# tspooner/rl_markets

Measured on NVIDIA H100. Metric: env steps/sec (batched LOBs), higher is better.
Workload: dtype f64

## Files before the change

rl_markets_b200/csrc/rlm_env.cuh:

```cuda
#pragma once
#include <cuda_runtime.h>
#include <math.h>
#include "rlm_types.h"

__constant__ DevParams P;

#define LLMIN ((long long)0x8000000000000000ull)
#ifdef RLM_ROLL_LEVELS
#define LEVEL_UNROLL _Pragma("unroll 1")
#else
#define LEVEL_UNROLL _Pragma("unroll")
#endif

__device__ __forceinline__ double pkey(double p) { return rint(p * 10000.0); }

__device__ __forceinline__ long long d2ll_x86(double d) {
  if (!(d >= -9223372036854775808.0 && d < 9223372036854775808.0)) return LLMIN;
  return (long long)d;
}

static_assert((RLM_MAX_BANDS & (RLM_MAX_BANDS - 1)) == 0, "the band search halves RLM_MAX_BANDS");
__device__ __noinline__ int to_ticks(double price, int* err, int* band_hint = nullptr) {
  const VenueD& V = P.venue;
  if (price < V.px[0]) { *err |= ERR_TICK_RANGE; return 0; }
  int k = 0;
  const int hk = band_hint ? *band_hint : -1;
  if ((unsigned)hk < (unsigned)(RLM_MAX_BANDS - 1) && !(price < V.px[hk]) && price < V.px[hk + 1]) {
    k = hk;
  } else {
#pragma unroll
    for (int step = RLM_MAX_BANDS / 2; step >= 1; step >>= 1)
      if (!(price < V.px[k + step])) k += step;
    if (band_hint) *band_hint = k;
  }
  int ticks = V.cum_full[k];
  double tsp = V.ts[k];
  int it = k;
#pragma unroll 1
  while (it < V.n && price + V.ts[it] / 2.0 > V.px[it]) {
    double ub;
    if (it == V.n - 1 || price < V.px[it + 1]) ub = price + tsp / 2.0;
    else ub = V.px[it + 1];
    const double inv = V.inv_ts[it];
    const double q = (inv != 0.0) ? (ub - V.px[it]) * inv : (ub - V.px[it]) / V.ts[it];
    ticks = (int)((double)ticks + q);
    ++it;
  }
  return ticks;
}

__device__ __noinline__ double to_price(int ticks, int* err) {
  const VenueD& V = P.venue;
  if (ticks < V.tts_tick[0]) { *err |= ERR_TICK_RANGE; return 0.0; }
  if (!(ticks > V.tts_tick[0])) return 0.0;
  int k = 0;
#pragma unroll
  for (int step = RLM_MAX_BANDS / 2; step >= 1; step >>= 1)
    if (ticks >= V.tts_tick[k + step]) k += step;
  double price = V.cum_price[k];
  if (ticks > V.tts_tick[k]) price += ((double)ticks - (double)V.tts_tick[k]) * V.ts[k];
  return price;
}

__device__ __forceinline__ bool market_is_open(const EnvHdr& e) {
  return ((long long)e.time_ms > P.venue.open_lo) && ((long long)e.time_ms < P.venue.close_hi);
}
__device__ __forceinline__ bool is_terminal(const EnvHdr& e) {
  return (!market_is_open(e)) || ((e.last_date != 0) && (e.date != e.last_date));
}

__device__ __forceinline__ long long ord_remaining(const OrderD& o) {
  long long r = o.size - o.executed;
  return r > 0 ? r : 0;
}
__device__ __forceinline__ bool ord_is_executed(const OrderD& o) { return o.executed >= o.size; }

__device__ __noinline__ long long ord_do_transaction(OrderD& o, long long volume) {
  o.transactions += (int)volume;
  long long remaining_volume = volume - o.q_head;
  if (remaining_volume > 0) {
    o.q_head = 0;
    if (ord_remaining(o) <= remaining_volume) {
      o.executed = o.size;
      remaining_volume -= o.size;
    } else {
      o.executed += remaining_volume;
      remaining_volume = 0;
    }
  } else {
    o.q_head -= volume;
  }
  return remaining_volume > 0 ? remaining_volume : 0;
}

__device__ __noinline__ void ord_do_cancellation(OrderD& o, long long volume) {
  if (o.q_tail == 0) {
    o.q_head -= volume;
  } else {
    double total = (double)(o.q_head + o.q_tail);
    o.q_head = d2ll_x86((double)o.q_head - ceil((double)(volume * o.q_head) / total));
    o.q_tail = d2ll_x86((double)o.q_tail - floor((double)(volume * o.q_tail) / total));
  }
  if (o.q_head < 0) {
    o.q_tail = (long long)((unsigned long long)o.q_tail + (unsigned long long)o.q_head);
    o.q_head = 0;
  }
  if (o.q_tail < 0) o.q_tail = 0;
}

__device__ long long side_volume(const SideD& s, double price) {
  if (!s.has_cur) return 0;
  double k = pkey(price);
  long long v = 0;
  LEVEL_UNROLL
  for (int l = 0; l < RLM_DEPTH; ++l)
    if (pkey(s.px[l]) == k) v = s.vol[l];
  return v;
}
__device__ long long side_last_volume(const SideD& s, double price) {
  if (!s.has_last) return 0;
  double k = pkey(price);
  long long v = 0;
  LEVEL_UNROLL
  for (int l = 0; l < RLM_DEPTH; ++l)
    if (pkey(s.last_px[l]) == k) v = s.last_vol[l];
  return v;
}

__device__ __noinline__ void side_reset(SideD& s) {
  s.n_transacted = 0; s.obs_value = 0.0; s.obs_volume = 0;
  s.total_vol = 0; s.last_total_vol = 0;
  for (int l = 0; l < RLM_DEPTH; ++l) { s.px[l] = 0.0; s.last_px[l] = 0.0; s.vol[l] = 0; s.last_vol[l] = 0; }
  s.has_cur = 0; s.has_last = 0;
  s.ord.live = 0;
}

__device__ __noinline__ void side_replace_order(SideD& s, double price, long long size, int* err) {
  if (price <= 0 || size <= 0) { *err |= ERR_BAD_PRICE; s.ord.live = 0; return; }
  OrderD& o = s.ord;
  o.live = 1; o.price = price; o.size = size;
  o.q_head = side_volume(s, price);
  o.q_tail = 0; o.executed = 0; o.transactions = 0; o.initial_queue = o.q_head;
}

__device__ __noinline__ void side_update_order(SideD& s, long long transaction_volume) {
  OrderD& o = s.ord;
  if (!o.live) return;
  if (ord_is_executed(o)) { o.live = 0; return; }
  long long lv = side_last_volume(s, o.price);
  if (lv == 0) return;
  long long v = side_volume(s, o.price);
  if (v == 0) { o.q_head = 0; o.q_tail = 0; return; }
  long long vol_diff = lv - v;
  if (vol_diff >= 0) {
    long long cancelled = vol_diff - transaction_volume;
    if (cancelled > 0) ord_do_cancellation(o, cancelled);
  } else {
    o.q_tail += vol_diff;
  }
}
// ... 135 lines not shown
}
__device__ __forceinline__ double win_back(const EnvHdr& e, const double* ring, int w) {
  int i = (e.w_count[w] == P.win_size[w]) ? e.w_head[w] : 0;
  return ring[P.win_off[w] + i];
}
__device__ __forceinline__ double win_std(const EnvHdr& e, int w) {
  double v = e.w_s[w] / (double)((unsigned long long)((long long)e.w_count[w] - 1));
  return v > 0 ? sqrt(v) : 0.0;
}

__device__ __noinline__ double get_reward(const EnvHdr& e) {
  double r = 0.0;
  long long ap = e.position < 0 ? -e.position : e.position;
  int abs_pos = (int)ap;
  switch (P.reward_measure) {
    case RLM_REWARD_NONE: break;
    case RLM_REWARD_PNL: r = e.pnl_step; break;
    case RLM_REWARD_PNL_DAMPED: r = e.pnl_step - (double)P.damping * fmax(0.0, e.momentum_pnl_step); break;
    case RLM_REWARD_SPREAD: r = e.pnl_step / e.w_mean[W_SPREAD]; break;
    case RLM_REWARD_NORMED:
      if (!(e.w_count[W_PNLUP] == P.win_size[W_PNLUP] && e.w_count[W_PNLDN] == P.win_size[W_PNLDN])) r = 0.0;
      else {
        double u = e.w_mean[W_PNLUP], d = e.w_mean[W_PNLDN];
        double su = win_std(e, W_PNLUP), sd = win_std(e, W_PNLDN);
        double numer = (u * sd - d * su), denom = (su + sd);
        if (isnan(numer) || isinf(numer)) numer = 0.0;
        if (isnan(denom) || isinf(denom)) denom = 0.0;
        r = (fabs(denom) < 1e-5) ? numer : (numer / denom);
      }
      break;
    case RLM_REWARD_LOVOL: r = (double)e.lo_vol_step; break;
    case RLM_REWARD_MM_LINEAR: r = (double)(-P.pos_weight * (float)abs_pos); r += (double)P.pnl_weight * e.pnl_step; break;
    case RLM_REWARD_MM_EXP:
      r = -pow(1.0 - exp((double)(P.pos_weight * (float)abs_pos)), 2.0); r += (double)P.pnl_weight * e.pnl_step; break;
    case RLM_REWARD_MM_DIV:
      if (e.pnl_step > 0) r = e.pnl_step / fmax(1.0, (double)abs_pos);
      else r = e.pnl_step;
      break;
  }
  return r * 100.0;
}

__device__ __noinline__ void clear_inventory(EnvHdr& e) {
  long long size = -e.position;
  Fill f; f.volume = 0; f.proxy = 0.0; f.value = 0.0;
  double mip = m_midprice(e);
  if (size > 0) f = side_walk<true>(e.side[0], mip, size);
  else if (size < 0) f = side_walk<false>(e.side[1], mip, size);
  e.position += f.volume;
  e.pnl_step += f.proxy;
  e.lo_vol_step += (int)(f.volume < 0 ? -f.volume : f.volume);
  e.ep_pnl += f.value;
  if (f.volume > 0) e.market_buys++;
  else if (f.volume < 0) e.market_sells++;
}

__device__ __noinline__ void place_orders(EnvHdr& e, int al, int bl) {
  e.ask_level = al; e.bid_level = bl;
  if (P.l2p_book) {
    e.ask_quote = to_price(to_ticks(e.side[0].px[0], &e.err, &e.tk_band) + al, &e.err);
    e.bid_quote = to_price(to_ticks(e.side[1].px[0], &e.err, &e.tk_band) - bl, &e.err);
  } else {
    double tp = e.tp_val, half_spd = fmax(0.0, e.w_mean[W_SPREAD] / 2.0);
    e.ask_quote = to_price(to_ticks(tp + (double)al * half_spd, &e.err, &e.tk_band), &e.err);
    e.bid_quote = to_price(to_ticks(tp - (double)bl * half_spd, &e.err, &e.tk_band), &e.err);
  }
  side_replace_order(e.side[0], e.ask_quote, P.order_size, &e.err);
  side_replace_order(e.side[1], e.bid_quote, P.order_size, &e.err);
}

__device__ __noinline__ void do_action(EnvHdr& e, int action) {
  int al, bl;
  switch (action) {
    case 0: al = 1; bl = 1; break;
    case 1: clear_inventory(e); al = e.ask_level; bl = e.bid_level; break;
    case 2: al = 2; bl = 2; break;
    case 3: al = 3; bl = 3; break;
    case 4: al = 0; bl = 2; break;
    case 5: al = 2; bl = 0; break;
    case 6: al = 1; bl = 4; break;
    case 7: al = 4; bl = 1; break;
    case 8: al = 5; bl = 5; break;
    default: return;
  }
  place_orders(e, al, bl);
}

__device__ __noinline__ void update_stats(EnvHdr& e) {
  e.ts_total++;
  bool has_ask = e.side[0].ord.live, has_bid = e.side[1].ord.live;
  if (has_ask) e.ts_ask++;
  if (has_bid) e.ts_bid++;
  if (has_ask && has_bid) e.ts_both++;
  if (e.position != 0) e.ts_pos++;
  if (e.position > 0) e.ts_long++;
  else if (e.position < 0) e.ts_short++;
}

__device__ __noinline__ void update_book_profiles(EnvHdr& e, const rlm_tick_msg& m) {
  e.last_date = e.date;
  e.date = m.date;
  e.time_ms = m.time_ms;
  side_apply_changes(e.side[0], m.ask_px, m.ask_vol, m, &e.err);
  side_apply_changes(e.side[1], m.bid_px, m.bid_vol, m, &e.err);
  if (e.side[0].has_last && e.side[1].has_last && !(pkey(e.side[0].last_px[0]) == 0.0) && !(pkey(e.side[1].last_px[0]) == 0.0)) {
    double mp = m_midprice(e);
    bool ok = (m_spread(e) >= 0.0) && (mp > 0.0) && (fabs(mp - m_last_midprice(e)) < mp);
    if (!ok) e.err |= ERR_INVALID_STATE;
  }
}

__device__ __noinline__ void next_state_tail(EnvHdr& e, const Fill& au, const Fill& bu, double* pushv) {
  Fill as = adverse_selection(e);
  e.pnl_step += au.proxy + bu.proxy + as.proxy;
  long long asabs = as.volume < 0 ? -as.volume : as.volume;
  e.lo_vol_step += (int)(bu.volume - au.volume + asabs);
  e.ep_pnl += au.value + bu.value + as.value;
  e.position += bu.volume + au.volume + as.volume;
  check_orders(e);
  double mid = m_midprice(e);
  long long mpt;
  if (mid == e.tk_px && mid > 0.0) mpt = e.tk_ticks;
  else { const int t = to_ticks(mid, &e.err, &e.tk_band); mpt = t; e.tk_px = mid; e.tk_ticks = t; }
  double mpm = mid - m_last_midprice(e), sp = m_spread(e);
  pushv[W_MID] = (double)mpt;
  pushv[W_VLT] = (double)mpt;
  pushv[W_VNUM] = e.side[0].obs_value + e.side[1].obs_value;
  pushv[W_VDEN] = (double)(e.side[0].obs_volume + e.side[1].obs_volume);
  pushv[W_SPREAD] = fmax(0.0, sp);
  pushv[W_TP] = P.tp_is_micro ? m_microprice(e) : mid;
  pushv[W_ASKTX] = (double)e.side[0].obs_volume;
  pushv[W_BIDTX] = (double)e.side[1].obs_volume;
  e.ewma_up = (P.ewma_alpha * fmax(0.0, mpm)) + ((1 - P.ewma_alpha) * e.ewma_up);
  e.ewma_dn = (P.ewma_alpha * fabs(fmin(0.0, mpm))) + ((1 - P.ewma_alpha) * e.ewma_dn);
  e.n_ticks++;
}

__device__ __forceinline__ void check_valid_state(EnvHdr& e) {
  if (e.side[0].has_last && e.side[1].has_last && !(pkey(e.side[0].last_px[0]) == 0.0) && !(pkey(e.side[1].last_px[0]) == 0.0)) {
    double mp = m_midprice(e);
    bool ok = (m_spread(e) >= 0.0) && (mp > 0.0) && (fabs(mp - m_last_midprice(e)) < mp);
    if (!ok) e.err |= ERR_INVALID_STATE;
  }
}

__device__ __noinline__ void next_state_scalar(EnvHdr& e, const rlm_tick_msg& m, double* pushv) {
  double mp = m_midprice(e);
  Fill au = side_apply_transactions<true>(e.side[0], m, mp, true);
  Fill bu = side_apply_transactions<false>(e.side[1], m, mp, true);
  update_book_profiles(e, m);
  next_state_tail(e, au, bu, pushv);
}

__device__ __noinline__ void next_state_warp(EnvHdr& e, const rlm_tick_msg& m, double* pushv, Fill* fills, int lane) {
  int* serr = (int*)(fills + 2);
  if (lane < 2) {
    const double mp = m_midprice(e);
    serr[lane] = 0;
    fills[lane] = (lane == 0) ? side_apply_transactions<true>(e.side[0], m, mp, true)
                              : side_apply_transactions<false>(e.side[1], m, mp, true);
  }
  __syncwarp();
  if (lane < 2) side_apply_changes(e.side[lane], lane == 0 ? m.ask_px : m.bid_px, lane == 0 ? m.ask_vol : m.bid_vol, m, &serr[lane]);
  __syncwarp();
  if (lane == 0) {
    e.last_date = e.date; e.date = m.date; e.time_ms = m.time_ms;
    e.err |= serr[0] | serr[1];
    check_valid_state(e);
    next_state_tail(e, fills[0], fills[1], pushv);
  }
}

__device__ __forceinline__ bool needs_multi(const EnvHdr& e, const rlm_tick_msg& m) { return (m.flags & 3) != 0 || e.tick_open != 0 || e.txn != 0; }
__device__ __forceinline__ void tick_tx_append(EnvHdr& e, const rlm_tick_msg& m) {
  for (int i = 0; i < m.n_tx && i < RLM_N_TX_MAX; ++i) {
    if (e.txn >= RLM_TX_CAP) { e.err |= ERR_BAD_PRICE; break; }
    e.tx_px[e.txn] = m.tx_px[i]; e.tx_vol[e.txn] = m.tx_vol[i]; e.txn++;
  }
}
__device__ __noinline__ bool update_book_profiles_multi(EnvHdr& e, const rlm_tick_msg& m, bool with_tx) {
  if (m.flags & RLM_TICK_TX_MORE) { if (with_tx && !e.tick_open) tick_tx_append(e, m); return false; }
  if (!e.tick_open) {
    if (with_tx) tick_tx_append(e, m); else e.txn = 0;
    side_stash(e.side[0]);
    side_stash(e.side[1]);
  }
  e.last_date = e.date;
  e.date = m.date;
  e.time_ms = m.time_ms;
  side_apply_row(e.side[0], m.ask_px, m.ask_vol, e.tx_px, e.tx_vol, e.txn, &e.err);
  side_apply_row(e.side[1], m.bid_px, m.bid_vol, e.tx_px, e.tx_vol, e.txn, &e.err);
  if (m.flags & RLM_TICK_PARTIAL) { e.tick_open = 1; return false; }
  e.tick_open = 0;
  e.txn = 0;
  return true;
}
__device__ __noinline__ bool next_state_multi(EnvHdr& e, const rlm_tick_msg& m, double* pushv) {
  if (m.flags & RLM_TICK_TX_MORE) { if (!e.tick_open) tick_tx_append(e, m); return false; }
  if (!e.tick_open) {
    tick_tx_append(e, m);
    const double mp = m_midprice(e);
    const Fill au = side_apply_transactions_n<true>(e.side[0], e.tx_px, e.tx_vol, e.txn, mp);
    const Fill bu = side_apply_transactions_n<false>(e.side[1], e.tx_px, e.tx_vol, e.txn, mp);
    e.tick_au.volume = au.volume; e.tick_au.proxy = au.proxy; e.tick_au.value = au.value;
    e.tick_bu.volume = bu.volume; e.tick_bu.proxy = bu.proxy; e.tick_bu.value = bu.value;
    side_stash(e.side[0]);
    side_stash(e.side[1]);
  }
  e.last_date = e.date;
  e.date = m.date;
  e.time_ms = m.time_ms;
  side_apply_row(e.side[0], m.ask_px, m.ask_vol, e.tx_px, e.tx_vol, e.txn, &e.err);
  side_apply_row(e.side[1], m.bid_px, m.bid_vol, e.tx_px, e.tx_vol, e.txn, &e.err);
  if (m.flags & RLM_TICK_PARTIAL) { e.tick_open = 1; return false; }
  e.tick_open = 0;
  e.txn = 0;
  check_valid_state(e);
  Fill au, bu;
  au.volume = e.tick_au.volume; au.proxy = e.tick_au.proxy; au.value = e.tick_au.value;
  bu.volume = e.tick_bu.volume; bu.proxy = e.tick_bu.proxy; bu.value = e.tick_bu.value;
  next_state_tail(e, au, bu, pushv);
  return true;
}

__device__ __forceinline__ double ulb_ref(double val, double lb, double ub) {
  const double m = (ub < val) ? ub : val;
  return (m < lb) ? lb : m;
}

__device__ __forceinline__ bool var_tick_args(const EnvHdr& e, const double* ring, int v, double& x0, double& x1) {
  switch (v) {
    case RLM_VAR_SPD: x0 = e.side[0].px[0]; x1 = e.side[1].px[0]; return true;
    case RLM_VAR_MPM: x0 = win_front(e, ring, W_MID); x1 = win_back(e, ring, W_MID); return true;
    case RLM_VAR_A_DIST: if (!e.side[0].ord.live) return false; x0 = e.side[0].ord.price; x1 = e.side[0].px[0]; return true;
    case RLM_VAR_B_DIST: if (!e.side[1].ord.live) return false; x0 = e.side[1].px[0]; x1 = e.side[1].ord.price; return true;
  }
  return false;
}
__device__ __forceinline__ double var_from_ticks(int v, int t0, int t1) {
  switch (v) {
    case RLM_VAR_SPD: return ulb_ref((double)(t0 - t1), 0.0, 20.0);
    case RLM_VAR_MPM: return ulb_ref((double)(t0 - t1), -10.0, 10.0);
  }
  return (double)t0 - (double)t1;
}

__device__ __noinline__ double get_variable(EnvHdr& e, const double* ring, int v) {
  switch (v) {
    case RLM_VAR_POS: return (double)e.position / (double)P.order_size;
    case RLM_VAR_SPD: {
      double d = (double)(to_ticks(e.side[0].px[0], &e.err, &e.tk_band) - to_ticks(e.side[1].px[0], &e.err, &e.tk_band));
      return ulb_ref(d, 0.0, 20.0);
    }
    case RLM_VAR_MPM: {
      double d = (double)(to_ticks(win_front(e, ring, W_MID), &e.err, &e.tk_band) - to_ticks(win_back(e, ring, W_MID), &e.err, &e.tk_band));
      return ulb_ref(d, -10.0, 10.0);
    }
    case RLM_VAR_IMB: {
      double v_a = (double)e.side[0].total_vol, v_b = (double)e.side[1].total_vol;
      return ((v_a + v_b) > 0 ? 5.0 * (v_b - v_a) / (v_b + v_a) : 0.0);
    }
    case RLM_VAR_SVL: {
      double q_a = e.w_sum[W_ASKTX], q_b = e.w_sum[W_BIDTX];
      return ((q_a + q_b) > 0 ? 5.0 * (q_b - q_a) / (q_a + q_b) : 0.0);
    }
    case RLM_VAR_VOL: return ulb_ref(5.0 * win_std(e, W_VLT), 0.0, 10.0);
    case RLM_VAR_RSI: {
      double u = e.ewma_up, d = e.ewma_dn;
      return (u + d) != 0.0 ? 5.0 * (u - d) / (u + d) : 0.0;
    }
    case RLM_VAR_VWAP: {
      double d = e.w_sum[W_VNUM] / e.w_sum[W_VDEN];
      return ulb_ref(d / e.w_mean[W_SPREAD], -10.0, 10.0);
    }
    case RLM_VAR_A_DIST:
      if (e.side[0].ord.live) return ((double)to_ticks(e.side[0].ord.price, &e.err, &e.tk_band) - (double)to_ticks(e.side[0].px[0], &e.err, &e.tk_band));
      else return -100.0;
    case RLM_VAR_A_QUEUE:
      if (e.side[0].ord.live) {
        float qp = (float)e.side[0].ord.q_head / fmaxf(1.0f, (float)e.side[0].ord.initial_queue);
        return 10.0 * (double)(long long)qp;
      } else return -1.0;
    case RLM_VAR_B_DIST:
      if (e.side[1].ord.live) return ((double)to_ticks(e.side[1].px[0], &e.err, &e.tk_band) - (double)to_ticks(e.side[1].ord.price, &e.err, &e.tk_band));
      else return -100.0;
    case RLM_VAR_B_QUEUE:
      if (e.side[1].ord.live) {
        float qp = (float)e.side[1].ord.q_head / fmaxf(1.0f, (float)e.side[1].ord.initial_queue);
        return 10.0 * (double)(long long)qp;
      } else return -1.0;
    case RLM_VAR_LAST_ACTION: return (double)e.last_action;
  }
  return 0.0;
}
```

rl_markets_b200/csrc/rlm_kernels.cu:

```cuda
#include <cuda_runtime.h>
#include <stdint.h>
#define RLM_TABLE_QUAL static __device__ const
#include "rlm_flow_tables.h"
#include "rlm_rndseq.h"
#include "rlm_agent.cuh"
#include <cstdio>
#include "rlm_kernels.h"
#define RLM_ENVT_CARVEOUT_DEFAULT 30
#define RLM_SMEM_CARVEOUT 88

#define SCR_Q 0
#define SCR_SS (SCR_Q + 8 * 2 * RLM_MAX_ACTIONS)
#define SCR_IDX (SCR_SS + 4 * SS_SLOTS)
#define SCR_VBUF (SCR_IDX + 4 * 3 * RLM_MAX_ACTIONS * 32)
#define AG_BYTES ((sizeof(AgentD) + 15) & ~(size_t)15)
size_t rlm_scratch_bytes(int is_double) {
  return ((size_t)SCR_VBUF + (size_t)(is_double ? 2 : 1) * RLM_MAX_ACTIONS * VROW * 8 + 15) & ~(size_t)15;
}
size_t rlm_agent_smem_bytes(int warps_per_cta, int scratch_bytes) {
  return (size_t)warps_per_cta * (AG_BYTES + (size_t)scratch_bytes);
}

#define PDL_PROLOGUE() do { asm volatile("griddepcontrol.launch_dependents;" ::: "memory"); asm volatile("griddepcontrol.wait;" ::: "memory"); } while (0)
static bool g_use_pdl = false;
// ... 423 lines not shown
  double pushv[RLM_NWIN], oldv[RLM_NWIN];
#pragma unroll
  for (int w = 0; w < RLM_NWIN; ++w) oldv[w] = window_peek(e, ring, w);
  if (phase == PH_RUN) e.pnl_step = 0.0;
  if (multi) { if (!next_state_multi(e, msg, pushv)) return -2; }
  else next_state_scalar(e, msg, pushv);
#pragma unroll 1
  for (int w = 0; w < 8; ++w) window_push(e, ring, w, pushv[w], oldv[w]);
  e.tp_val = e.w_mean[W_TP];
  if (phase == PH_WARMUP) {
    bool full = true;
#pragma unroll 1
    for (int w = 0; w < 8; ++w) full = full && (e.w_count[w] == P.win_size[w]);
    if (!full) return -1;
    place_orders(e, 1, 1);
    e.phase = PH_RUN;
    e.ag.kind = 1;
    if (backtest) {
#pragma unroll 1
      for (int i = 0; i < P.n_state_vars; ++i) e.ag.to_vars[i] = (float)get_variable(e, ring, P.state_vars[i]);
    }
    return 1;
  }
  double mpm = m_midprice(e) - m_last_midprice(e);
  e.pnl_step += (double)e.position * mpm;
  e.momentum_pnl_step += (double)e.position * mpm;
  e.agg_r += get_reward(e);
  e.agg_pnl += e.pnl_step;
  e.agg_mpm += mpm;
  if (!is_terminal(e) && fabs(e.agg_mpm) < 1e-5) return -1;
  e.pnl_step = e.agg_pnl;
  window_push(e, ring, W_PNLUP, fmax(0.0, e.pnl_step), oldv[W_PNLUP]);
  window_push(e, ring, W_PNLDN, fabs(fmin(0.0, e.pnl_step)), oldv[W_PNLDN]);
  e.ep_reward += e.agg_r;
  e.ep_bandh += e.agg_mpm;
#pragma unroll 1
  for (int i = 0; i < P.n_state_vars; ++i) e.ag.to_vars[i] = (float)get_variable(e, ring, P.state_vars[i]);
  e.ag.last_reward = get_reward(e);
  e.ag.kind = 0;
  e.ag.hs_valid = 0;
  return 0;
}

template <int THREADS>
__global__ void __launch_bounds__(THREADS) rlm_env_kernel(DevPtrs ptr, DynParams D, int tslot, int only_begin) {
  const int b = D.env0 + blockIdx.x * THREADS + threadIdx.x;
  const int lane = threadIdx.x & 31;
  if (!only_begin) KLOG_BEGIN(0);
  int ready = -1;
  unsigned ticked = 0, errs = 0;
  if (b < (D.n_sub > 0 ? D.env0 + D.n_sub : P.n_envs)) {
    EnvHdr* g = (EnvHdr*)(ptr.env + (size_t)b * P.env_stride);
    const int ph = g->phase;
    const int nb = D.hold ? 0 : g->ag.need_begin;
    if (ph != PH_DONE && (!only_begin || nb) && !(D.hold && env_on_hold(*g))) {
      EnvHdr e;
      constexpr int HOT16 = (int)(offsetof(EnvHdr, ag) / 16), ALL16 = (int)(sizeof(EnvHdr) / 16);
      static_assert(offsetof(EnvHdr, ag) % 16 == 0 && sizeof(EnvHdr) % 16 == 0, "16-byte copies of the two halves of the record");
      bool ag_in = nb || D.hold || D.backtest;
      {
        const int4* src = (const int4*)g;
        int4* dst = (int4*)&e;
        for (int i = 0; i < HOT16; ++i) dst[i] = src[i];
        if (ag_in) for (int i = HOT16; i < ALL16; ++i) dst[i] = src[i];
        else e.ag.err = 0;
      }
      double* ring = (double*)((unsigned char*)g + sizeof(EnvHdr));
      if (nb) {
        begin_step(e, ptr.mt_pol + (size_t)b * 312, D);
        e.ag.need_begin = 0;
      }
      if (!only_begin && e.phase != PH_DONE) {
        rlm_tick_msg msg;
        bool have = true;
        if (P.source == RLM_SOURCE_GENERATOR) {
          flow_next_dev(&e.flow, &msg);
        } else {
          const rlm_tick_msg* sp = ptr.stream;
          int s_off = D.stream_off, s_n = D.stream_ticks;
          if (D.ctl_stream) {
            const int4 rc4 = __ldg((const int4*)ptr.runctl);
            s_off = rc4.z; s_n = rc4.w;
            sp = (const rlm_tick_msg*)__ldg((const unsigned long long*)ptr.runctl + 2);
          }
          const int pos = s_off + tslot;
          if (pos >= s_n) { e.err |= ERR_STREAM_UNDERRUN; have = false; }
          else {
            const int4* src = (const int4*)(sp + ((size_t)pos * P.n_envs + b));
            int4* dst = (int4*)&msg;
#pragma unroll
            for (int i = 0; i < 8; ++i) dst[i] = __ldg(src + i);
          }
        }
        if (have) {
          const int was = e.phase;
          ready = env_tick(e, ring, msg, D.backtest);
          if (was != PH_PREOPEN && ready != -2) ticked = 1;
          if (ready == -2) ready = -1;
        }
      }
      if (ready >= 0 && !ag_in) {
        const int kind = e.ag.kind;
        const double rew = e.ag.last_reward;
        float tv[RLM_N_STATE_MAX];
        for (int i = 0; i < RLM_N_STATE_MAX; ++i) tv[i] = (i < P.n_state_vars) ? e.ag.to_vars[i] : 0.0f;
        const int4* src = (const int4*)g;
        int4* dst = (int4*)&e;
        for (int i = HOT16; i < ALL16; ++i) dst[i] = src[i];
        e.ag.kind = kind;
        if (kind == 0) {
          e.ag.last_reward = rew; e.ag.hs_valid = 0;
          for (int i = 0; i < RLM_N_STATE_MAX; ++i) if (i < P.n_state_vars) e.ag.to_vars[i] = tv[i];
        }
        ag_in = true;
      }
      errs = (unsigned)(e.err | e.ag.err);
      {
        int4* dst = (int4*)g;
        const int4* src = (const int4*)&e;
        for (int i = 0; i < HOT16; ++i) dst[i] = src[i];
        if (ag_in) for (int i = HOT16; i < ALL16; ++i) dst[i] = src[i];
      }
    }
  }
  if (D.hold) {
    bool still = false;
    if (b < (D.n_sub > 0 ? D.env0 + D.n_sub : P.n_envs) && ready < 0 && !only_begin) {
      const EnvHdr* g = (const EnvHdr*)(ptr.env + (size_t)b * P.env_stride);
      still = g->phase != PH_DONE && !env_on_hold(*g);
    }
    const unsigned rm = __ballot_sync(FULL, still);
    if (rm && lane == 0) atomicAdd(&ptr.counters[5], (unsigned long long)__popc(rm));
  }
  const unsigned m = __ballot_sync(FULL, ready >= 0);
  if (m) {
    const int leader = __ffs(m) - 1;
    int base = 0;
    if (lane == leader) base = atomicAdd(&ptr.ready_count[tslot], __popc(m));
    base = __shfl_sync(FULL, base, leader);
    if (ready >= 0) ptr.ready[base + __popc(m & ((1u << lane) - 1u))] = b;
  }
  if (!only_begin) KLOG_END(0);
  const unsigned tm = __ballot_sync(FULL, ticked != 0);
  unsigned em = errs;
  for (int o = 16; o > 0; o >>= 1) em |= __shfl_xor_sync(FULL, em, o);
  if (lane == 0) {
    if (tm) atomicAdd(&ptr.counters[0], (unsigned long long)__popc(tm));
    if (em) atomicOr(&ptr.counters[4], (unsigned long long)em);
  }
}

#define ENVW_WARPS 8
#define ENVW_WARPS_DEFAULT 8
__host__ __device__ inline size_t envw_hdr_bytes() { return (sizeof(EnvHdr) + 15) & ~(size_t)15; }
__host__ __device__ inline size_t envw_warp_bytes() { return envw_hdr_bytes() + 128 + 8 * 2 * RLM_NWIN + 128; }
struct EnvWarp {
  EnvHdr* e; rlm_tick_msg* msg; double* pushv; double* oldv; int* flag; unsigned* r12; Fill* fills;
};
__device__ __forceinline__ EnvWarp envw_carve(unsigned char* wbase) {
  EnvWarp w;
  const size_t hb = envw_hdr_bytes();
  w.e = (EnvHdr*)wbase;
  w.msg = (rlm_tick_msg*)(wbase + hb);
  w.pushv = (double*)(wbase + hb + 128);
  w.oldv = w.pushv + RLM_NWIN;
  w.flag = (int*)(w.oldv + RLM_NWIN);
  w.r12 = (unsigned*)(w.flag + 4);
  w.fills = (Fill*)(w.r12 + 12);
  return w;
}
__device__ __forceinline__ void envw_stage_in(EnvHdr* dst_e, const EnvHdr* g, int lane) {
  const int4* src = (const int4*)g;
  int4* dst = (int4*)dst_e;
  const int n16 = (int)(envw_hdr_bytes() / 16);
  static_assert(sizeof(EnvHdr) <= 4 * 32 * 16, "four 16-byte loads per lane cover the env header");
  int4 t[4];
#pragma unroll
  for (int k = 0; k < 4; ++k) { const int i = lane + 32 * k; if (i < n16) t[k] = src[i]; }
#pragma unroll
  for (int k = 0; k < 4; ++k) { const int i = lane + 32 * k; if (i < n16) dst[i] = t[k]; }
}
__device__ __forceinline__ void envw_stage_out(EnvHdr* g, const EnvHdr* src_e, int lane) {
  int4* dst = (int4*)g;
  const int4* src = (const int4*)src_e;
  for (int i = lane; i < (int)(envw_hdr_bytes() / 16); i += 32) dst[i] = src[i];
}

__device__ __forceinline__ int envw_tick(const EnvWarp& w, double* ring, const DevPtrs& ptr, const DynParams& D, int env, int stream_pos,
                                         int stream_ticks, int lane, unsigned& ticked) {
  EnvHdr& e = *w.e;
  rlm_tick_msg& msg = *w.msg;
  double* pushv = w.pushv;
  double* oldv = w.oldv;
  int ready = -1;
  bool have = true;
  if (P.source == RLM_SOURCE_GENERATOR) {
    flow_next_warp(&e.flow, &msg, w.r12, lane);
  } else {
    if (stream_pos >= stream_ticks) { if (lane == 0) e.err |= ERR_STREAM_UNDERRUN; have = false; }
    else ((unsigned*)&msg)[lane] = __ldg((const unsigned*)(ptr.stream + ((size_t)stream_pos * P.n_envs + env)) + lane);
  }
  if (lane < RLM_NWIN) oldv[lane] = window_peek(e, ring, lane);
  __syncwarp();
  const int phase = e.phase;
  const bool multi = have && needs_multi(e, msg);
  int complete = 1;
  if (multi && phase != PH_PREOPEN) {
    if (lane == 0) {
      if (phase == PH_RUN) e.pnl_step = 0.0;
      complete = next_state_multi(e, msg, pushv) ? 1 : 0;
    }
    complete = __shfl_sync(FULL, complete, 0);
  }
  if (have && phase == PH_PREOPEN) {
    if (lane == 0) {
      if (multi) {
        if (update_book_profiles_multi(e, msg, false) && market_is_open(e)) e.phase = PH_WARMUP;
      } else {
        msg.n_tx = 0;
        update_book_profiles(e, msg);
        if (market_is_open(e)) e.phase = PH_WARMUP;
      }
    }
  } else if (have && complete) {
    ticked += 1;
    if (!multi) {
      if (lane == 0 && phase == PH_RUN) e.pnl_step = 0.0;
      __syncwarp();
      next_state_warp(e, msg, pushv, w.fills, lane);
    }
    __syncwarp();
    if (lane < 8) window_push(e, ring, lane, pushv[lane], oldv[lane]);
    __syncwarp();
    if (lane == 0) {
      int r = -1;
      e.tp_val = e.w_mean[W_TP];
      if (phase == PH_WARMUP) {
        bool full = true;
        for (int k = 0; k < 8; ++k) full = full && (e.w_count[k] == P.win_size[k]);
        if (full) {
          place_orders(e, 1, 1);
          e.phase = PH_RUN;
          e.ag.kind = 1;
          r = 1;
        }
      } else {
        double mpm = m_midprice(e) - m_last_midprice(e);
        e.pnl_step += (double)e.position * mpm;
        e.momentum_pnl_step += (double)e.position * mpm;
        e.agg_r += get_reward(e);
        e.agg_pnl += e.pnl_step;
        e.agg_mpm += mpm;
        if (!(!is_terminal(e) && fabs(e.agg_mpm) < 1e-5)) {
          e.pnl_step = e.agg_pnl;
          pushv[W_PNLUP] = fmax(0.0, e.pnl_step);
          pushv[W_PNLDN] = fabs(fmin(0.0, e.pnl_step));
          e.ep_reward += e.agg_r;
          e.ep_bandh += e.agg_mpm;
          r = 0;
        }
      }
      *w.flag = r;
    }
    __syncwarp();
    ready = *w.flag;
    if (ready == 0) {
      if (lane == W_PNLUP || lane == W_PNLDN) window_push(e, ring, lane, pushv[lane], oldv[lane]);
      __syncwarp();
      {
        const bool has = lane < P.n_state_vars;
        const int var = has ? P.state_vars[lane] : -1;
        double x0 = 0.0, x1 = 0.0;
        const bool two = has && var_tick_args(e, ring, var, x0, x1);
        int t0 = 0, t1 = 0, lerr = 0, hint = e.tk_band;
        if (two) { t0 = to_ticks(x0, &lerr, &hint); t1 = to_ticks(x1, &lerr, &hint); }
        if (lerr) atomicOr(&e.err, lerr);
        if (has) e.ag.to_vars[lane] = (float)(two ? var_from_ticks(var, t0, t1) : get_variable(e, ring, var));
      }
      if (lane == 31) { e.ag.last_reward = get_reward(e); e.ag.kind = 0; }
      if (D.env_hash && !D.backtest && !P.shared_policy && P.algorithm < RLM_ALGO_R_LEARN) {
        __syncwarp();
        const LnSums h = ln_hash(rlm_rndseq_table, e.ag.to_vars, false, lane);
        unsigned long long* hs = ptr.hsum + (size_t)env * 96;
        hs[lane] = h.s[0]; hs[32 + lane] = h.s[1]; hs[64 + lane] = h.s[2];
        const double* th_a = ptr.theta + (size_t)env * (size_t)P.memory_size;
        const double* th_b = ptr.theta_b ? ptr.theta_b + (size_t)env * (size_t)P.memory_size : nullptr;
#pragma unroll 1
        for (int g = 0; g < 3; ++g) {
#pragma unroll
          for (int a = 0; a < RLM_MAX_ACTIONS; ++a) {
            if (a < P.n_actions) {
              const int f = mod_m(h.s[g] + P.rg[g][a]);
              asm volatile("prefetch.global.L2 [%0];" ::"l"(th_a + f));
              if (th_b) asm volatile("prefetch.global.L2 [%0];" ::"l"(th_b + f));
            }
          }
        }
        if (lane == 0) e.ag.hs_valid = 1;
      }
    } else if (ready == 1 && D.backtest) {
      if (lane < P.n_state_vars) e.ag.to_vars[lane] = (float)get_variable(e, ring, P.state_vars[lane]);
    }
  }
  __syncwarp();
  return ready;
}

__global__ void __launch_bounds__(ENVW_WARPS * 32) rlm_env_kernel_w(DevPtrs ptr, DynParams D, int tslot, int only_begin) {
  PDL_PROLOGUE();
  extern __shared__ __align__(16) unsigned char smem[];
  const int tid = threadIdx.x, lane = tid & 31, warp = tid >> 5;
  const int env = D.env0 + blockIdx.x * (blockDim.x >> 5) + warp;
  if (!only_begin) KLOG_BEGIN(0);
  if (env >= (D.n_sub > 0 ? D.env0 + D.n_sub : P.n_envs)) return;
  const EnvWarp w = envw_carve(smem + (size_t)warp * envw_warp_bytes());
  EnvHdr& e = *w.e;
  EnvHdr* g = (EnvHdr*)(ptr.env + (size_t)env * P.env_stride);
  double* ring = (double*)((unsigned char*)g + sizeof(EnvHdr));
  if (only_begin && !g->ag.need_begin) return;
  envw_stage_in(&e, g, lane);
  __syncwarp();
  if (e.phase == PH_DONE) return;
  if (D.hold && env_on_hold(e)) return;
  int ready = -1;
  unsigned ticked = 0;
  if (e.ag.need_begin) begin_step_warp(e, ptr.mt_pol + (size_t)env * 312, D, w.flag, lane);
  if (!only_begin && e.phase != PH_DONE) {
    if (D.ctl_stream) {
      const int4 rc4 = __ldg((const int4*)ptr.runctl);
      DevPtrs pt = ptr;
      pt.stream = (const rlm_tick_msg*)__ldg((const unsigned long long*)ptr.runctl + 2);
      ready = envw_tick(w, ring, pt, D, env, rc4.z + tslot, rc4.w, lane, ticked);
    } else {
      ready = envw_tick(w, ring, ptr, D, env, D.stream_off + tslot, D.stream_ticks, lane, ticked);
    }
  }
  __syncwarp();
  envw_stage_out(g, &e, lane);
  if (!only_begin) KLOG_END(0);
  if (lane == 0) {
    if (ready >= 0) ptr.ready[atomicAdd(&ptr.ready_count[tslot], 1)] = env;
    if (D.hold && ready < 0 && e.phase != PH_DONE) atomicAdd(&ptr.counters[5], 1ull);
    if (ticked) atomicAdd(&ptr.counters[0], 1ull);
    const unsigned errs = (unsigned)(e.err | e.ag.err);
    if (errs) atomicOr(&ptr.counters[4], (unsigned long long)errs);
  }
}

__global__ void __launch_bounds__(ENVW_WARPS * 32, 4) rlm_env_round_kernel(DevPtrs ptr, DynParams D, int tslot) {
  PDL_PROLOGUE();
  extern __shared__ __align__(16) unsigned char smem[];
  const int tid = threadIdx.x, lane = tid & 31, warp = tid >> 5;
  const int env = D.env0 + blockIdx.x * (blockDim.x >> 5) + warp;
  KLOG_BEGIN(0);
  if (env >= (D.n_sub > 0 ? D.env0 + D.n_sub : P.n_envs)) return;
  int* live_count = ptr.ready_count + RLM_LIVE_OFF;
  if (tslot > 0 && __ldcg(live_count + tslot - 1) == 0) return;
  const int4 rc4 = __ldg((const int4*)ptr.runctl);
  const RunCtl rc = {rc4.x, rc4.y, rc4.z, rc4.w, nullptr, 0};
  DevPtrs pt = ptr;
  pt.stream = (const rlm_tick_msg*)__ldg((const unsigned long long*)ptr.runctl + 2);
  const EnvWarp w = envw_carve(smem + (size_t)warp * envw_warp_bytes());
  EnvHdr& e = *w.e;
  EnvHdr* g = (EnvHdr*)(ptr.env + (size_t)env * P.env_stride);
  double* ring = (double*)((unsigned char*)g + sizeof(EnvHdr));
  envw_stage_in(&e, g, lane);
  __syncwarp();
  if (e.phase == PH_DONE) return;
  int pos = e.run_id == rc.run_id ? e.run_pos : 0;
  if (pos >= rc.n_ticks && !e.ag.need_begin) return;
  int ready = -1;
  unsigned ticked = 0;
  const int cap = D.round_cap > 0 ? D.round_cap : 0x7fffffff;
  int n_run = 0;
#pragma unroll 1
  for (;;) {
    if (e.ag.need_begin) begin_step_warp(e, ptr.mt_pol + (size_t)env * 312, D, w.flag, lane);
    if (e.phase == PH_DONE || pos >= rc.n_ticks || n_run >= cap) break;
    ready = envw_tick(w, ring, pt, D, env, rc.stream_off + pos, rc.stream_ticks, lane, ticked);
    ++pos; ++n_run;
    if (ready >= 0) break;
  }
  if (lane == 0) { e.run_id = rc.run_id; e.run_pos = pos; }
  __syncwarp();
  envw_stage_out(g, &e, lane);
  KLOG_END(0);
  if (lane == 0) {
    if (ready >= 0) ptr.ready[atomicAdd(&ptr.ready_count[tslot], 1)] = env;
    if (ready >= 0 || (e.phase != PH_DONE && pos < rc.n_ticks)) atomicAdd(&live_count[tslot], 1);
    if (ticked) atomicAdd(&ptr.counters[0], (unsigned long long)ticked);
    const unsigned errs = (unsigned)(e.err | e.ag.err);
    if (errs) atomicOr(&ptr.counters[4], (unsigned long long)errs);
  }
}
__global__ void rlm_runctl_kernel(RunCtl* dst, RunCtl v) { *dst = v; }

__device__ __forceinline__ void emit_record(const DevPtrs& ptr, const EnvHdr* g, int env, const AgentD& ag, const double* theta_a,
                                         const float* vars, int lane) {
  const int* tf = ptr.trace_f + (size_t)env * P.trace_cap;
  const float* te = ptr.trace_e + (size_t)env * P.trace_cap;
  unsigned long long h = trace_hash(tf, te, theta_a, ag.n_traces, lane);
  if (lane == 0) {
    int c = ptr.record_count[env];
    if (c < P.record_cap) {
      EnvHdr tmp;
      const int4* src = (const int4*)g;
      int4* dst = (int4*)&tmp;
      for (int i = 0; i < (int)(sizeof(EnvHdr) / 16); ++i) dst[i] = __ldcg(src + i);
      fill_record(&ptr.records[(size_t)env * P.record_cap + c], tmp, ag, h, vars);
    }
    ptr.record_count[env] = c + 1;
  }
}

__device__ __noinline__ void emit_record_ool(const DevPtrs& ptr, const EnvHdr* g, int env, const AgentD& ag, const double* theta_a,
                                             const float* vars, int lane) {
  emit_record(ptr, g, env, ag, theta_a, vars, lane);
}
__device__ __noinline__ void emit_record_res(const DevPtrs& ptr, const EnvHdr* e, int env, const AgentD& ag, const double* theta_a,
                                             const float* vars, int lane) {
  const int* tf = ptr.trace_f + (size_t)env * P.trace_cap;
  const float* te = ptr.trace_e + (size_t)env * P.trace_cap;
  const unsigned long long h = trace_hash(tf, te, theta_a, ag.n_traces, lane);
  if (lane == 0) {
    const int c = ptr.record_count[env];
    if (c < P.record_cap) fill_record(&ptr.records[(size_t)env * P.record_cap + c], *e, ag, h, vars);
    ptr.record_count[env] = c + 1;
  }
}

__device__ __forceinline__ void backtest_advance(const DevPtrs& ptr, const EnvHdr* g, int env, AgentD& ag, const double* theta_a,
                                                 int kind, double qa, double qb, unsigned long long base0, int lane,
                                                 unsigned long long& steps_done) {
  if (kind == 0) {
    if (lane == 0) ag.last_delta = 0.0;
    __syncwarp();
    if (env < P.record_envs) emit_record_ool(ptr, g, env, ag, theta_a, ag.from_vars, lane);
    __syncwarp();
  }
  if (lane < P.n_actions) { ag.q_from[lane] = qa; ag.qb_from[lane] = qb; }
  if (lane < RLM_N_STATE_MAX + 3) ag.from_vars[lane] = ag.to_vars[lane];
  ag.from_base0[lane] = mod_m(base0);
  if (lane == 0) {
    ag.null_from = 0; ag.need_begin = 1;
    if (kind == 0) { ag.n_steps++; ag.ep_step++; } else ag.kind = 2;
  }
  if (kind == 0) steps_done++;
}

__device__ __noinline__ void td_decision(AgentD& ag, const double* q_pre_a, const double* q_pre_b, unsigned long long* mt_pol,
                                         unsigned long long* mt_agt, const DynParams& D, double* out) {
  ASSUME_SHARED(&ag); ASSUME_SHARED(q_pre_a); ASSUME_SHARED(q_pre_b); ASSUME_SHARED(out); ASSUME_GLOBAL(mt_pol);
  const int action = ag.cur_action;
  const double reward = ag.last_reward;
  const double F_term = P.gamma * 0.0 - 0.0;
  float rate = P.gl;
  double delta;
  int table = 0;
  if (P.algorithm == RLM_ALGO_SARSA) {
    double Q1 = ag.q_from[action];
    int a2 = policy_action(ag, q_pre_a, q_pre_b, mt_pol, D);
    double Q2 = q_pre_a[a2];
    delta = reward + F_term + P.gamma * Q2 - Q1;
  } else if (P.algorithm == RLM_ALGO_Q_LEARN) {
    int amax = argmax_ties_fast(ag, ag.q_from);
    if (action != amax) rate = 0.0f;
    double Q = ag.q_from[action];
    int am2 = argmax_ties_fast(ag, q_pre_a);
    delta = reward + F_term + P.gamma * q_pre_a[am2] - Q;
  } else if (P.algorithm == RLM_ALGO_DOUBLE_Q_LEARN) {
    int amax = argmax_ties_fast(ag, ag.q_from);
    if (action != amax) rate = 0.0f;
    if (mt_uniform_real(mt_agt, ag.mt_agt_idx) > 0.5) {
      double Qa = ag.q_from[action];
      int am2 = argmax_ties_fast(ag, q_pre_a);
      delta = reward + F_term + P.gamma * q_pre_b[am2] - Qa;
      table = 0;
    } else {
      double Qb = ag.qb_from[action];
      int am2 = argmax_ties_fast(ag, q_pre_b);
      delta = reward + F_term + P.gamma * q_pre_a[am2] - Qb;
      table = 1;
    }
  } else if (P.algorithm == RLM_ALGO_R_LEARN) {
    int amax = argmax_ties_fast(ag, ag.q_from);
    if (action != amax) rate = 0.0f;
    double Q = ag.q_from[action];
    double mQ = q_pre_a[argmax_ties_fast(ag, q_pre_a)];
    delta = reward - ag.rho + mQ - Q;
    out[3] = Q; out[4] = mQ;
  } else if (P.algorithm == RLM_ALGO_ONLINE_R_LEARN) {
    double Q = ag.q_from[action];
    double gQ = q_pre_a[policy_action(ag, q_pre_a, q_pre_b, mt_pol, D)];
    delta = reward - ag.rho + gQ - Q;
    out[3] = Q; out[4] = gQ;
  } else {
    int amax = argmax_ties_fast(ag, ag.q_from);
    if (action != amax) rate = 0.0f;
    double Q, mQ;
    if (mt_uniform_real(mt_agt, ag.mt_agt_idx) > 0.5) {
      Q = ag.q_from[action];
      mQ = q_pre_b[argmax_ties_fast(ag, q_pre_a)];
      table = 0;
    } else {
      Q = ag.qb_from[action];
      mQ = q_pre_a[argmax_ties_fast(ag, q_pre_b)];
      table = 1;
    }
    delta = reward - ag.rho + mQ - Q;
    out[3] = Q; out[4] = mQ;
  }
  ag.last_delta = delta;
  out[0] = (double)rate;
  out[1] = (D.alpha * delta) * (1.0 / (double)RLM_N_TILINGS);
  out[2] = (double)table;
}

__device__ __noinline__ void td_rho(AgentD& ag, const double* q_post_a, const double* q_post_b, const DynParams& D, const double* dec) {
  const double Q = dec[3];
  double boot = dec[4];
  const double nQ = Q + D.alpha * ag.last_delta;
  double best;
  if (P.algorithm == RLM_ALGO_DOUBLE_R_LEARN) {
    best = -1.7976931348623157e308;
    for (int i = 0; i < P.n_actions; i++) {
      double val = (q_post_a[i] + q_post_b[i]) / 2.0;
      if (val > best) best = val;
    }
    boot = best;
  } else {
    best = q_post_a[argmax_ties(ag, q_post_a)];
  }
  if (nQ - best < 1e-7) ag.rho += P.beta * (ag.last_reward - ag.rho + boot - nQ);
}

#ifdef RLM_TIMING
__device__ long long g_phase_clk[4096 * 16];
__device__ unsigned g_phase_sm[4096];
// ... 951 lines not shown
```

Baseline: 12.34 million.

## Parallelize book-level change application across warp lanes in next_state_warp

Replaces the two-lane serial side_apply_changes with a 16-lane version where each lane handles one depth level per side, using ballots and shuffles to locate the order's price level in the old book, new book and transactions. Transaction application gets a lead-lane fast path that only accumulates observed value and volume, and calls the full routine only when the live order could be reached. It also adds compile-time-gated per-phase clock64 timing instrumentation, which is off by default. The rewritten change logic must exactly reproduce the original semantics (error flags, cancellations, queue updates), so it risks subtle divergence.

New measurement: 12.48 million (median of 6 runs). +1.1%, better.

```diff
diff --git a/rl_markets_b200/csrc/rlm_env.cuh b/rl_markets_b200/csrc/rlm_env.cuh
--- a/rl_markets_b200/csrc/rlm_env.cuh
+++ b/rl_markets_b200/csrc/rlm_env.cuh
@@ -6,6 +6,16 @@
 __constant__ DevParams P;
 
 #define LLMIN ((long long)0x8000000000000000ull)
+
+#ifdef RLM_TIMING
+#define TPH(clk, i) do { if (lane == 0) { const long long t_ = clock64(); (clk)[i] += t_ - (clk)[15]; (clk)[15] = t_; } } while (0)
+#define TPH_COUNT(clk, i) do { if (lane == 0) (clk)[i] += 1; } while (0)
+#else
+#define TPH(clk, i) do { } while (0)
+#define TPH_COUNT(clk, i) do { } while (0)
+#endif
+enum { TPH_STAGE_IN = 0, TPH_BEGIN, TPH_GEN, TPH_APPLY_TX, TPH_APPLY_CHANGES, TPH_TAIL, TPH_WINDOWS, TPH_STEP_END, TPH_STAGE_OUT,
+       TPH_N_TICKS, TPH_N_LAUNCHES };
 #ifdef RLM_ROLL_LEVELS
 #define LEVEL_UNROLL _Pragma("unroll 1")
 #else
@@ -447,23 +457,95 @@
   next_state_tail(e, au, bu, pushv);
 }
 
-__device__ __noinline__ void next_state_warp(EnvHdr& e, const rlm_tick_msg& m, double* pushv, Fill* fills, int lane) {
-  int* serr = (int*)(fills + 2);
-  if (lane < 2) {
-    const double mp = m_midprice(e);
-    serr[lane] = 0;
-    fills[lane] = (lane == 0) ? side_apply_transactions<true>(e.side[0], m, mp, true)
-                              : side_apply_transactions<false>(e.side[1], m, mp, true);
-  }
+
+__device__ __forceinline__ Fill side_transactions_lead(SideD& s, bool ask, const rlm_tick_msg& m, double ref) {
+  const int n = m.n_tx;
+  const double op = s.ord.price;
+  double value = 0.0;
+  long long volume = 0;
+  bool reach = false;
+#pragma unroll 1
+  for (int k = 0; k < n; ++k) {
+    const int i = ask ? k : n - 1 - k;
+    const double tp = (double)m.tx_px[i];
+    if (ask ? (tp < ref) : (tp > ref)) continue;
+    const long long vol = m.tx_vol[i];
+    value += tp * (double)vol;
+    volume += vol;
+    reach = reach || (ask ? (op <= tp) : (op >= tp));
+  }
+  if (reach && s.ord.live) return ask ? side_apply_transactions<true>(s, m, ref, true) : side_apply_transactions<false>(s, m, ref, true);
+  s.obs_value = value;
+  s.obs_volume = volume;
+  Fill f; f.volume = 0; f.proxy = 0.0; f.value = 0.0;
+  return f;
+}
+
+__device__ __noinline__ void next_state_warp(EnvHdr& e, const rlm_tick_msg& m, double* pushv, Fill* fills, int lane, long long* clk) {
+  constexpr unsigned FULL = 0xffffffffu;
+  const int s = (lane >> 3) & 1, l = lane & 7;
+  const bool book = lane < 16, lead = book && l == 0, level = book && l < RLM_DEPTH;
+  SideD& sd = e.side[s];
+  if (lead) fills[s] = side_transactions_lead(sd, s == 0, m, m_midprice(e));
   __syncwarp();
-  if (lane < 2) side_apply_changes(e.side[lane], lane == 0 ? m.ask_px : m.bid_px, lane == 0 ? m.ask_vol : m.bid_vol, m, &serr[lane]);
+  TPH(clk, TPH_APPLY_TX);
+  double opx = 0.0, npx = 0.0;
+  int ovol = 0, nvol = 0, tvol = 0;
+  if (level) {
+    opx = sd.px[l]; ovol = sd.vol[l];
+    npx = (double)(s == 0 ? m.ask_px : m.bid_px)[l];
+    nvol = (s == 0 ? m.ask_vol : m.bid_vol)[l];
+    sd.last_px[l] = opx; sd.last_vol[l] = ovol;
+    sd.px[l] = npx; sd.vol[l] = nvol;
+  }
+  const unsigned bad = __ballot_sync(FULL, level && (npx <= 0.0 || nvol <= 0));
+  long long tv = nvol;
+  tv += __shfl_xor_sync(FULL, tv, 1);
+  tv += __shfl_xor_sync(FULL, tv, 2);
+  tv += __shfl_xor_sync(FULL, tv, 4);
+  const double k = pkey(sd.ord.price);
+  const bool tx = book && l < m.n_tx;
+  if (tx) tvol = m.tx_vol[l];
+  const unsigned ml = __ballot_sync(FULL, level && pkey(opx) == k);
+  const unsigned mc = __ballot_sync(FULL, level && pkey(npx) == k);
+  const unsigned mt = __ballot_sync(FULL, tx && pkey((double)m.tx_px[l]) == k);
+  const int sh = 8 * s;
+  const unsigned bl = (ml >> sh) & 0xFFu, bc = (mc >> sh) & 0xFFu, bt = (mt >> sh) & 0xFFu;
+  const int lv = __shfl_sync(FULL, ovol, bl ? sh + 31 - __clz(bl) : lane);
+  const int v = __shfl_sync(FULL, nvol, bc ? sh + 31 - __clz(bc) : lane);
+  const int t = __shfl_sync(FULL, tvol, bt ? sh + 31 - __clz(bt) : lane);
+  if (lead) {
+    const int had = sd.has_cur;
+    sd.has_last = had;
+    sd.last_total_vol = sd.total_vol;
+    sd.total_vol += tv;
+    sd.has_cur = 1;
+    OrderD& o = sd.ord;
+    if (o.live) {
+      if (ord_is_executed(o)) o.live = 0;
+      else if (had && bl && lv != 0) {
+        if (!bc || v == 0) { o.q_head = 0; o.q_tail = 0; }
+        else {
+          const long long vol_diff = (long long)lv - (long long)v;
+          if (vol_diff >= 0) {
+            const long long cancelled = vol_diff - (long long)(bt ? t : 0);
+            if (cancelled > 0) ord_do_cancellation(o, cancelled);
+          } else {
+            o.q_tail += vol_diff;
+          }
+        }
+      }
+    }
+  }
   __syncwarp();
+  TPH(clk, TPH_APPLY_CHANGES);
   if (lane == 0) {
     e.last_date = e.date; e.date = m.date; e.time_ms = m.time_ms;
-    e.err |= serr[0] | serr[1];
+    if (bad) e.err |= ERR_BAD_PRICE;
     check_valid_state(e);
     next_state_tail(e, fills[0], fills[1], pushv);
   }
+  TPH(clk, TPH_TAIL);
 }
 
 __device__ __forceinline__ bool needs_multi(const EnvHdr& e, const rlm_tick_msg& m) { return (m.flags & 3) != 0 || e.tick_open != 0 || e.txn != 0; }
diff --git a/rl_markets_b200/csrc/rlm_kernels.cu b/rl_markets_b200/csrc/rlm_kernels.cu
--- a/rl_markets_b200/csrc/rlm_kernels.cu
+++ b/rl_markets_b200/csrc/rlm_kernels.cu
@@ -599,10 +599,26 @@
 
 #define ENVW_WARPS 8
 #define ENVW_WARPS_DEFAULT 8
+#ifdef RLM_TIMING
+#define ENVW_CLK_BYTES 128
+__device__ long long g_tick_clk[4096 * 16];
+extern "C" int rlm_debug_read_tick_phases(long long* clk, int reset) {
+  if (cudaDeviceSynchronize() != cudaSuccess) return -1;
+  if (clk && cudaMemcpyFromSymbol(clk, g_tick_clk, sizeof(g_tick_clk)) != cudaSuccess) return -1;
+  if (reset) {
+    static long long zero[4096 * 16];
+    if (cudaMemcpyToSymbol(g_tick_clk, zero, sizeof(zero)) != cudaSuccess) return -1;
+  }
+  return 0;
+}
+#else
+#define ENVW_CLK_BYTES 0
+#endif
 __host__ __device__ inline size_t envw_hdr_bytes() { return (sizeof(EnvHdr) + 15) & ~(size_t)15; }
-__host__ __device__ inline size_t envw_warp_bytes() { return envw_hdr_bytes() + 128 + 8 * 2 * RLM_NWIN + 128; }
+__host__ __device__ inline size_t envw_warp_bytes() { return envw_hdr_bytes() + 128 + 8 * 2 * RLM_NWIN + 128 + ENVW_CLK_BYTES; }
 struct EnvWarp {
   EnvHdr* e; rlm_tick_msg* msg; double* pushv; double* oldv; int* flag; unsigned* r12; Fill* fills;
+  long long* clk;
 };
 __device__ __forceinline__ EnvWarp envw_carve(unsigned char* wbase) {
   EnvWarp w;
@@ -614,8 +630,16 @@
   w.flag = (int*)(w.oldv + RLM_NWIN);
   w.r12 = (unsigned*)(w.flag + 4);
   w.fills = (Fill*)(w.r12 + 12);
+  w.clk = ENVW_CLK_BYTES ? (long long*)(wbase + hb + 128 + 8 * 2 * RLM_NWIN + 128) : nullptr;
   return w;
 }
+#ifdef RLM_TIMING
+#define TPH_START(w) do { if (lane < 16) (w).clk[lane] = 0; __syncwarp(); if (lane == 0) (w).clk[15] = clock64(); } while (0)
+#define TPH_FLUSH(w, env) do { __syncwarp(); if ((env) < 4096 && lane < 15) g_tick_clk[(env) * 16 + lane] += (w).clk[lane]; } while (0)
+#else
+#define TPH_START(w) do { } while (0)
+#define TPH_FLUSH(w, env) do { } while (0)
+#endif
 __device__ __forceinline__ void envw_stage_in(EnvHdr* dst_e, const EnvHdr* g, int lane) {
   const int4* src = (const int4*)g;
   int4* dst = (int4*)dst_e;
@@ -649,6 +673,7 @@
   }
   if (lane < RLM_NWIN) oldv[lane] = window_peek(e, ring, lane);
   __syncwarp();
+  TPH(w.clk, TPH_GEN);
   const int phase = e.phase;
   const bool multi = have && needs_multi(e, msg);
   int complete = 1;
@@ -674,9 +699,10 @@
     if (!multi) {
       if (lane == 0 && phase == PH_RUN) e.pnl_step = 0.0;
       __syncwarp();
-      next_state_warp(e, msg, pushv, w.fills, lane);
+      next_state_warp(e, msg, pushv, w.fills, lane, w.clk);
     }
     __syncwarp();
+    TPH(w.clk, TPH_TAIL);
     if (lane < 8) window_push(e, ring, lane, pushv[lane], oldv[lane]);
     __syncwarp();
     if (lane == 0) {
@@ -711,6 +737,7 @@
     }
     __syncwarp();
     ready = *w.flag;
+    TPH(w.clk, TPH_WINDOWS);
     if (ready == 0) {
       if (lane == W_PNLUP || lane == W_PNLDN) window_push(e, ring, lane, pushv[lane], oldv[lane]);
       __syncwarp();
@@ -748,6 +775,9 @@
     } else if (ready == 1 && D.backtest) {
       if (lane < P.n_state_vars) e.ag.to_vars[lane] = (float)get_variable(e, ring, P.state_vars[lane]);
     }
+    __syncwarp();
+    TPH(w.clk, TPH_STEP_END);
+    TPH_COUNT(w.clk, TPH_N_TICKS);
   }
   __syncwarp();
   return ready;
@@ -765,13 +795,17 @@
   EnvHdr* g = (EnvHdr*)(ptr.env + (size_t)env * P.env_stride);
   double* ring = (double*)((unsigned char*)g + sizeof(EnvHdr));
   if (only_begin && !g->ag.need_begin) return;
+  TPH_START(w);
   envw_stage_in(&e, g, lane);
   __syncwarp();
   if (e.phase == PH_DONE) return;
   if (D.hold && env_on_hold(e)) return;
+  TPH(w.clk, TPH_STAGE_IN);
+  TPH_COUNT(w.clk, TPH_N_LAUNCHES);
   int ready = -1;
   unsigned ticked = 0;
   if (e.ag.need_begin) begin_step_warp(e, ptr.mt_pol + (size_t)env * 312, D, w.flag, lane);
+  TPH(w.clk, TPH_BEGIN);
   if (!only_begin && e.phase != PH_DONE) {
     if (D.ctl_stream) {
       const int4 rc4 = __ldg((const int4*)ptr.runctl);
@@ -784,6 +818,8 @@
   }
   __syncwarp();
   envw_stage_out(g, &e, lane);
+  TPH(w.clk, TPH_STAGE_OUT);
+  TPH_FLUSH(w, env);
   if (!only_begin) KLOG_END(0);
   if (lane == 0) {
     if (ready >= 0) ptr.ready[atomicAdd(&ptr.ready_count[tslot], 1)] = env;
@@ -811,11 +847,14 @@
   EnvHdr& e = *w.e;
   EnvHdr* g = (EnvHdr*)(ptr.env + (size_t)env * P.env_stride);
   double* ring = (double*)((unsigned char*)g + sizeof(EnvHdr));
+  TPH_START(w);
   envw_stage_in(&e, g, lane);
   __syncwarp();
   if (e.phase == PH_DONE) return;
   int pos = e.run_id == rc.run_id ? e.run_pos : 0;
   if (pos >= rc.n_ticks && !e.ag.need_begin) return;
+  TPH(w.clk, TPH_STAGE_IN);
+  TPH_COUNT(w.clk, TPH_N_LAUNCHES);
   int ready = -1;
   unsigned ticked = 0;
   const int cap = D.round_cap > 0 ? D.round_cap : 0x7fffffff;
@@ -823,6 +862,7 @@
 #pragma unroll 1
   for (;;) {
     if (e.ag.need_begin) begin_step_warp(e, ptr.mt_pol + (size_t)env * 312, D, w.flag, lane);
+    TPH(w.clk, TPH_BEGIN);
     if (e.phase == PH_DONE || pos >= rc.n_ticks || n_run >= cap) break;
     ready = envw_tick(w, ring, pt, D, env, rc.stream_off + pos, rc.stream_ticks, lane, ticked);
     ++pos; ++n_run;
@@ -831,6 +871,8 @@
   if (lane == 0) { e.run_id = rc.run_id; e.run_pos = pos; }
   __syncwarp();
   envw_stage_out(g, &e, lane);
+  TPH(w.clk, TPH_STAGE_OUT);
+  TPH_FLUSH(w, env);
   KLOG_END(0);
   if (lane == 0) {
     if (ready >= 0) ptr.ready[atomicAdd(&ptr.ready_count[tslot], 1)] = env;
```
